# zhaoyuhsin/Edge-Guided-Near-Eye-Image-Analysis-for-Head-Mounted-Displays

Measured on AMD Instinct MI355X. Metric: eye-frames/sec (320x240): inference edge+seg (value), +fit, exact fp32, and train fwd+bwd at 1 MI355X, higher is better.
Workload: dtype f32 tensors; inference products split into f16 hi/lo pairs (3 f16 MFMAs per product, 22-bit significand), f32 accumulate (`exact_fp32`: every product on the f32 MFMA); `train`: bf16 storage, f32 accumulate, f32 master weights (and an f32-storage leg)

## Files before the change

edge-guided-near-eye-image-analysis-for-head-mounted-displays_amd/csrc/common.h:

```cpp
#pragma once
#include <hip/hip_runtime.h>
#include <cstdarg>
#include <cstdio>
#include <mutex>
#include <unordered_map>
#include "../../include/egne_hip.h"

static __device__ __attribute__((aligned(256), used)) float egne_zero_page[64] = {0};

typedef __bf16 egne_bf16;
typedef float egne_f32x4 __attribute__((ext_vector_type(4)));
typedef __bf16 egne_bf16x4 __attribute__((ext_vector_type(4)));
typedef __bf16 egne_bf16x8 __attribute__((ext_vector_type(8)));

__device__ __forceinline__ egne_f32x4 ld4(const float* p) { return *(const egne_f32x4*)p; }
__device__ __forceinline__ egne_f32x4 ld4(const egne_bf16* p) { return __builtin_convertvector(*(const egne_bf16x4*)p, egne_f32x4); }
__device__ __forceinline__ void st4(float* p, egne_f32x4 v) { *(egne_f32x4*)p = v; }
__device__ __forceinline__ void st4(egne_bf16* p, egne_f32x4 v) { *(egne_bf16x4*)p = __builtin_convertvector(v, egne_bf16x4); }
__device__ __forceinline__ float ld1(const float* p) { return *p; }
__device__ __forceinline__ float ld1(const egne_bf16* p) { return (float)*p; }
__device__ __forceinline__ void st1(float* p, float v) { *p = v; }
__device__ __forceinline__ void st1(egne_bf16* p, float v) { *p = (egne_bf16)v; }
template <typename T> struct egne_vt { static constexpr int N = 4; };
template <> struct egne_vt<egne_bf16> { static constexpr int N = 8; };
template <int N> struct egne_fv { float v[N]; };
__device__ __forceinline__ egne_fv<4> ldv(const float* p) {
  const egne_f32x4 t = *(const egne_f32x4*)p;
  return egne_fv<4>{{t[0], t[1], t[2], t[3]}};
}
__device__ __forceinline__ egne_fv<8> ldv(const egne_bf16* p) {
  typedef unsigned u4_ __attribute__((ext_vector_type(4)));
  const u4_ w = *(const u4_*)p;
  egne_fv<8> r;
#pragma unroll
  for (int i = 0; i < 4; ++i) {
    r.v[2 * i] = __builtin_bit_cast(float, w[i] << 16);
    r.v[2 * i + 1] = __builtin_bit_cast(float, w[i] & 0xffff0000u);
  }
  return r;
}
__device__ __forceinline__ void stv(float* p, const egne_fv<4>& a) { *(egne_f32x4*)p = egne_f32x4{a.v[0], a.v[1], a.v[2], a.v[3]}; }
__device__ __forceinline__ void stv(egne_bf16* p, const egne_fv<8>& a) {
  const egne_f32x4 lo = {a.v[0], a.v[1], a.v[2], a.v[3]}, hi = {a.v[4], a.v[5], a.v[6], a.v[7]};
  const egne_bf16x4 l = __builtin_convertvector(lo, egne_bf16x4), h = __builtin_convertvector(hi, egne_bf16x4);
  *(egne_bf16x8*)p = egne_bf16x8{l[0], l[1], l[2], l[3], h[0], h[1], h[2], h[3]};
}
typedef unsigned egne_u32x4 __attribute__((ext_vector_type(4)));
template <typename T> __device__ __forceinline__ egne_u32x4 ldraw(const T* p) { return *(const egne_u32x4*)p; }
__device__ __forceinline__ egne_fv<4> unpackv(const float*, egne_u32x4 w) {
  return egne_fv<4>{{__builtin_bit_cast(float, w[0]), __builtin_bit_cast(float, w[1]), __builtin_bit_cast(float, w[2]), __builtin_bit_cast(float, w[3])}};
}
__device__ __forceinline__ egne_fv<8> unpackv(const egne_bf16*, egne_u32x4 w) {
  egne_fv<8> r;
#pragma unroll
  for (int i = 0; i < 4; ++i) {
    r.v[2 * i] = __builtin_bit_cast(float, w[i] << 16);
    r.v[2 * i + 1] = __builtin_bit_cast(float, w[i] & 0xffff0000u);
  }
  return r;
}
template <int N> __device__ __forceinline__ egne_fv<N> ldf(const float* p) {
  egne_fv<N> r;
#pragma unroll
  for (int i = 0; i < N; i += 4) { const egne_f32x4 t = *(const egne_f32x4*)(p + i); r.v[i] = t[0]; r.v[i + 1] = t[1]; r.v[i + 2] = t[2]; r.v[i + 3] = t[3]; }
  return r;
}
template <int N> __device__ __forceinline__ egne_fv<N> fv_fill(float x) {
  egne_fv<N> r;
#pragma unroll
  for (int i = 0; i < N; ++i) r.v[i] = x;
  return r;
}
template <typename T> __device__ __forceinline__ const T* zero_page() { return (const T*)egne_zero_page; }

#ifdef EGNE_NO_OVF_CHECK
__device__ __forceinline__ bool egne_nonfinite(float) { return false; }
__device__ __forceinline__ bool egne_nonfinite64(double) { return false; }
#else
__device__ __forceinline__ bool egne_nonfinite(float v) { return __builtin_amdgcn_classf(v, 0x207); }
__device__ __forceinline__ bool egne_nonfinite64(double v) { return !__builtin_isfinite(v); }
#endif
__device__ __forceinline__ bool egne_ovf_row(int y, int H) { return y % 3 == 1 || y == H - 1; }
__device__ __forceinline__ void egne_ovf_commit(bool bad, unsigned* flag) {
  if (flag && bad) atomicOr(flag, 1u);
}

namespace egne {

char* err_buf();

inline int fail(int code, const char* fmt, ...) {
  va_list ap;
  va_start(ap, fmt);
  vsnprintf(err_buf(), 512, fmt, ap);
  va_end(ap);
  return code;
}

inline bool fp32_storage(const egne_conv_desc& d) {
  for (int i = 0; i < d.nseg && i < EGNE_MAXSEG; ++i)
    if (d.seg[i].presplit != 0) return false;
  return d.out_split == 0;
}

inline int check_launch(const char* what) {
  hipError_t e = hipGetLastError();
  if (e != hipSuccess) return fail(EGNE_ERR_LAUNCH, "%s: %s", what, hipGetErrorString(e));
  return EGNE_OK;
}

inline bool raise_lds(const void* kern, size_t bytes) {
  static std::mutex mu;
  static std::unordered_map<const void*, size_t> have;
  std::lock_guard<std::mutex> g(mu);
  auto it = have.find(kern);
  if (it != have.end() && it->second >= bytes) return true;
  if (hipFuncSetAttribute(kern, hipFuncAttributeMaxDynamicSharedMemorySize, (int)bytes) != hipSuccess) {
    (void)hipGetLastError();
    return false;
  }
  have[kern] = bytes;
  return true;
}
template <typename... K> inline bool raise_lds_all(size_t bytes, K... kern) { return (raise_lds((const void*)kern, bytes) && ...); }

#define EGNE_REQUIRE(cond, ...) \
  do { if (!(cond)) return ::egne::fail(EGNE_ERR_ARG, __VA_ARGS__); } while (0)

bool halo3_supported(const egne_conv_desc& d);
int halo3_launch(const egne_conv_desc& d, hipStream_t st);

bool wgrad_halo_supported(const egne_conv_desc& d, long long gzs);
int wgrad_halo_splits(const egne_conv_desc& d);
int wgrad_halo_launch(const egne_conv_desc& d, const float* gz, long long gzs, int gzo, float* ws, hipStream_t st);
int wgrad_halo_f16_launch(const egne_conv_desc& d, const float* gz, long long gzs, int gzo, const unsigned* gz_dyn, float* ws, hipStream_t st);

bool wgrad3x3_bf16_supported(const egne_conv_desc& d, long long gzs);
int wgrad3x3_bf16_splits(const egne_conv_desc& d);
int wgrad3x3_bf16_launch(const egne_conv_desc& d, const egne_bf16* gz, long long gzs, int gzo, float* ws, hipStream_t st);
bool wgrad1x1_bf16_supported(const egne_conv_desc& d, long long gzs);
int wgrad1x1_bf16_splits(const egne_conv_desc& d);
int wgrad1x1_bf16_launch(const egne_conv_desc& d, const egne_bf16* gz, long long gzs, int gzo, float* ws, hipStream_t st);

inline int cdiv(long long a, long long b) { return (int)((a + b - 1) / b); }

}
```

edge-guided-near-eye-image-analysis-for-head-mounted-displays_amd/csrc/conv_f16x3_big.hip:

```cpp
#include "common.h"
#include "kernel_util.h"
#include "split_f16.h"
#include <cstdlib>
#include <type_traits>

namespace {

constexpr int BM = 256, ROWB = 128;

template <int NB, bool M16, int NP = 3, int PS = 0>
__global__ __launch_bounds__(512) void conv_f16x3_big_kernel(const egne_conv_desc p, const char* __restrict__ wimg, float a_scale,
                                                             float out_scale) {
  constexpr int BN = 128 * NB;
  constexpr int STAGE = (BM + BN) * ROWB;
  extern __shared__ __attribute__((aligned(1024))) char lds[];
  const int tid = threadIdx.x, lane = tid & 63;
  const int wave = (PS & 2) ? __builtin_amdgcn_readfirstlane(tid >> 6) : tid >> 6;
  const int wm = wave >> 2, wn = wave & 3;
  const long long M = (long long)p.B * p.Ho * p.Wo;
  const long long m0 = (long long)blockIdx.x * BM;
  const int ntile = blockIdx.y;
  const int T = p.kh * p.kw;
  const egne_seg sg = p.seg[0];
  const int hw = p.Ho * p.Wo, frame_px = p.H * p.W;
  const int b0 = (int)(m0 / hw);
  const long long in_left = ((long long)p.B - b0) * frame_px * sg.pix_stride * 4;
  const __amdgpu_buffer_rsrc_t rin = make_rsrc(sg.ptr + (long long)b0 * frame_px * sg.pix_stride,
                                               (unsigned)(in_left < 0x7fffffffll ? in_left : 0x7fffffffll));
  const int nchunk = sg.Cp >> 5;
  const int nsteps = T * nchunk;
  const __amdgpu_buffer_rsrc_t rw = make_rsrc(wimg + (long long)ntile * nsteps * (BN * ROWB), (unsigned)(nsteps * BN * ROWB));

  const int c4 = tid & 7;
  int roff[4];
  unsigned tapmask[4];
  {
    const int dil = p.dil[0];
#pragma unroll
    for (int i = 0; i < 4; ++i) {
      const int row_i = (PS & 2) ? 32 * wave + 8 * i + (lane >> 3) : (tid >> 3) + 64 * i;
      const long long m = m0 + row_i;
      const int b = (int)(m / hw);
      const int r = (int)(m - (long long)b * hw);
      const int oy = r / p.Wo, ox = r - oy * p.Wo;
      const int lc = (lane & 7) ^ (((row_i >> 1) + 6) & 7);
      roff[i] = ((((b - b0) * p.H + oy) * p.W + ox) * (int)sg.pix_stride + sg.ch_off) * 4 + ((PS & 2) ? (lc & 1) * 64 + (lc >> 1) * 16 : c4 * 16);
      unsigned mk = 0;
      for (int ky = 0; ky < p.kh; ++ky)
        for (int kx = 0; kx < p.kw; ++kx) {
          const int iy = oy + (ky - p.pad_h) * dil, ix = ox + (kx - p.pad_w) * dil;
          if (m < M && iy >= 0 && iy < p.H && ix >= 0 && ix < p.W) mk |= 1u << (ky * p.kw + kx);
        }
      tapmask[i] = mk;
    }
  }
  int ldst_hi[4], ldst_lo[4];
#pragma unroll
  for (int i = 0; i < 4; ++i) {
    const int r = (tid >> 3) + 64 * i, g = c4 >> 1, sw = ((r >> 1) + 6) & 7;
    ldst_hi[i] = r * ROWB + (((2 * g) ^ sw) << 4) + (c4 & 1) * 8;
    ldst_lo[i] = r * ROWB + (((2 * g + 1) ^ sw) << 4) + (c4 & 1) * 8;
  }
  const int wvoff = lane * 16;

  u32x4 ra[4];
  int ky_n = 0, kx_n = 0, c0_n = 0;
  auto load_a = [&](int tap, int stage) {
    const int dil = p.dil[0];
    const int tapoff = (((ky_n - p.pad_h) * p.W + (kx_n - p.pad_w)) * dil * (int)sg.pix_stride + c0_n) * 4;
#pragma unroll
    for (int i = 0; i < 4; ++i) {
      const bool ok = (tapmask[i] >> tap) & 1u;
      if constexpr ((PS & 2))
        __builtin_amdgcn_raw_ptr_buffer_load_lds(rin, (lds_ptr)(lds + stage * STAGE + wave * 4096 + i * 1024), 16, ok ? roff[i] + tapoff : (int)OOB, 0, 0, 0);
      else
        ra[i] = __builtin_amdgcn_raw_buffer_load_b128(rin, ok ? roff[i] + tapoff : (int)OOB, 0, 0);
    }
  };
  auto dma_b = [&](int stage, int step) {
    char* base = lds + stage * STAGE + BM * ROWB;
#pragma unroll
    for (int j = 0; j < 2 * NB; ++j) {
      const int blk = wave * 2 * NB + j;
      __builtin_amdgcn_raw_ptr_buffer_load_lds(rw, (lds_ptr)(base + blk * 1024), 16, wvoff, step * (BN * ROWB) + blk * 1024, 0, 0);
    }
  };
  auto store_a = [&](int stage) {
    char* base = lds + stage * STAGE;
#pragma unroll
    for (int i = 0; i < ((PS & 2) ? 0 : 4); ++i) {
      const f32x4 v = __builtin_bit_cast(f32x4, ra[i]);
      if constexpr (NP == 1) {
        const f32x2 t0 = {v[0] * a_scale, v[1] * a_scale}, t1 = {v[2] * a_scale, v[3] * a_scale};
        const h2 h0 = __builtin_convertvector(t0, h2), h1 = __builtin_convertvector(t1, h2);
        const h4 hi = {h0[0], h0[1], h1[0], h1[1]};
        *(h4*)(base + ldst_hi[i]) = hi;
        continue;
      }
      h2 h0, h1, l0, l1;
      egne::split2(v[0], v[1], a_scale, h0, l0);
      egne::split2(v[2], v[3], a_scale, h1, l1);
      const h4 hi = {h0[0], h0[1], h1[0], h1[1]}, lo = {l0[0], l0[1], l1[0], l1[1]};
      *(h4*)(base + ldst_hi[i]) = hi;
      *(h4*)(base + ldst_lo[i]) = lo;
    }
  };
  auto advance = [&]() {
    if (++kx_n == p.kw) { kx_n = 0; ++ky_n; }
    if (ky_n == p.kh) { ky_n = 0; c0_n += 32; }
  };

  constexpr int MB = M16 ? 16 : 32, NTM = 128 / MB, NTN = 32 * NB / MB;
  using acc_t = std::conditional_t<M16, f32x4, f32x16>;
  acc_t acc[NTM][NTN];
#pragma unroll
  for (int a = 0; a < NTM; ++a)
#pragma unroll
    for (int b = 0; b < NTN; ++b) acc[a][b] = (acc_t)(0.f);

  const int lr = lane & (MB - 1), kg = lane / MB;
  int aoffs[NTM], boffs[NTN];
#pragma unroll
  for (int t = 0; t < NTM; ++t) aoffs[t] = (wm * 128 + t * MB + lr) * ROWB;
#pragma unroll
  for (int t = 0; t < NTN; ++t) boffs[t] = BM * ROWB + (wn * 32 * NB + t * MB + lr) * ROWB;
  const int sw = ((lr >> 1) + 6) & 7;

  load_a(0, 0);
  dma_b(0, 0);
  store_a(0);
  advance();
  asm volatile("s_waitcnt vmcnt(0) lgkmcnt(0)" ::: "memory");
  __builtin_amdgcn_s_barrier();

  int tap_n = 1 % T;
  for (int step = 0; step < nsteps; ++step) {
    const int st = step & 1;
    const bool more = step + 1 < nsteps;
    if (more) {
      load_a(tap_n, st ^ 1);
      dma_b(st ^ 1, step + 1);
    }
    const char* base = lds + st * STAGE;
    if constexpr (M16) {
      const int ch = ((2 * kg) ^ sw) << 4, cl = ((2 * kg + 1) ^ sw) << 4;
      h8 bh[NTN], bl[NTN];
#pragma unroll
      for (int t = 0; t < NTN; ++t) {
        bh[t] = *(const h8*)(base + boffs[t] + ch);
        if constexpr (NP == 3) bl[t] = *(const h8*)(base + boffs[t] + cl);
      }
#pragma unroll
      for (int half = 0; half < 2; ++half) {
        h8 ah[4], al[4];
#pragma unroll
        for (int t = 0; t < 4; ++t) {
          ah[t] = *(const h8*)(base + aoffs[half * 4 + t] + ch);
          if constexpr (NP == 3) al[t] = *(const h8*)(base + aoffs[half * 4 + t] + cl);
        }
#pragma unroll
        for (int t = 0; t < 4; ++t)
#pragma unroll
          for (int tn = 0; tn < NTN; ++tn) {
            acc_t& c = acc[half * 4 + t][tn];
            if constexpr (NP == 3) {
              c = __builtin_amdgcn_mfma_f32_16x16x32_f16(bh[tn], al[t], c, 0, 0, 0);
              c = __builtin_amdgcn_mfma_f32_16x16x32_f16(bl[tn], ah[t], c, 0, 0, 0);
            }
            c = __builtin_amdgcn_mfma_f32_16x16x32_f16(bh[tn], ah[t], c, 0, 0, 0);
          }
      }
    } else {
#pragma unroll
    for (int ks = 0; ks < 2; ++ks) {
      const int ch = ((2 * (2 * ks + kg)) ^ sw) << 4, cl = ((2 * (2 * ks + kg) + 1) ^ sw) << 4;
      h8 ah[4], al[4], bh[NB], bl[NB];
#pragma unroll
      for (int t = 0; t < 4; ++t) {
        ah[t] = *(const h8*)(base + aoffs[t] + ch);
        al[t] = *(const h8*)(base + aoffs[t] + cl);
      }
#pragma unroll
      for (int t = 0; t < NB; ++t) {
        bh[t] = *(const h8*)(base + boffs[t] + ch);
        bl[t] = *(const h8*)(base + boffs[t] + cl);
      }
#pragma unroll
      for (int tm = 0; tm < 4; ++tm)
#pragma unroll
        for (int tn = 0; tn < NB; ++tn) {
          if constexpr (!M16) {
            acc[tm][tn] = __builtin_amdgcn_mfma_f32_32x32x16_f16(bh[tn], al[tm], acc[tm][tn], 0, 0, 0);
            acc[tm][tn] = __builtin_amdgcn_mfma_f32_32x32x16_f16(bl[tn], ah[tm], acc[tm][tn], 0, 0, 0);
            acc[tm][tn] = __builtin_amdgcn_mfma_f32_32x32x16_f16(bh[tn], ah[tm], acc[tm][tn], 0, 0, 0);
          }
        }
    }
    }
    if (more) {
      store_a(st ^ 1);
      advance();
      tap_n = tap_n + 1 == T ? 0 : tap_n + 1;
    }
    asm volatile("s_waitcnt vmcnt(0) lgkmcnt(0)" ::: "memory");
    __builtin_amdgcn_s_barrier();
  }

  const float slope = p.act == EGNE_ACT_RELU ? 0.f : (p.act == EGNE_ACT_LEAKY ? 0.01f : 1.f);
  const long long left = M - m0;
  const __amdgpu_buffer_rsrc_t rout = make_rsrc(p.out + m0 * p.out_pix_stride, (unsigned)((left < BM ? left : BM) * p.out_pix_stride * 4));
  constexpr int NJ = M16 ? 1 : 4;
  bool bad = false;
  if constexpr (PS & 1) {
    static_assert(M16 && NP == 3, "split-pair output: 16 x 16 x 32 shape, three products");
    const float oss = p.out_split_scale;
    const bool odd = kg & 1;
    const int pb = (odd ? 32 : 0) + 16 * (kg >> 1);
#pragma unroll
    for (int bp = 0; bp < NTN / 2; ++bp) {
      const int nb = ntile * BN + wn * 32 * NB + bp * 32;
      const bool nok = nb < p.Cout_store;
      const f32x4 bv0 = (p.bias && nok) ? *(const f32x4*)(p.bias + nb + 4 * kg) : (f32x4)(0.f);
      const f32x4 bv1 = (p.bias && nok) ? *(const f32x4*)(p.bias + nb + 16 + 4 * kg) : (f32x4)(0.f);
#pragma unroll
      for (int tm = 0; tm < NTM; ++tm) {
        u32x2 hi[2], lo[2];
#pragma unroll
        for (int q = 0; q < 2; ++q) {
          f32x4 v;
#pragma unroll
          for (int e = 0; e < 4; ++e) {
            const float t = acc[tm][2 * bp + q][e] * out_scale + (q ? bv1[e] : bv0[e]);
            v[e] = fmaxf(t, t * slope);
          }
          h2 h0, h1, l0, l1;
          egne::split2(v[0], v[1], oss, h0, l0);
          egne::split2(v[2], v[3], oss, h1, l1);
          if (bp == 0 && q == 0) bad |= egne_nonfinite(v[0]) || egne_nonfinite((float)h0[0]);
          hi[q] = u32x2{__builtin_bit_cast(unsigned, h0), __builtin_bit_cast(unsigned, h1)};
          lo[q] = u32x2{__builtin_bit_cast(unsigned, l0), __builtin_bit_cast(unsigned, l1)};
        }
        const u32x2 sh = odd ? hi[0] : hi[1], sl = odd ? lo[0] : lo[1];
        u32x2 rh, rl;
#pragma unroll
        for (int e = 0; e < 2; ++e) {
          rh[e] = (unsigned)__builtin_amdgcn_ds_swizzle((int)sh[e], 0x401f);
          rl[e] = (unsigned)__builtin_amdgcn_ds_swizzle((int)sl[e], 0x401f);
        }
        const u32x4 oh = odd ? u32x4{rh[0], rh[1], hi[1][0], hi[1][1]} : u32x4{hi[0][0], hi[0][1], rh[0], rh[1]};
        const u32x4 ol = odd ? u32x4{rl[0], rl[1], lo[1][0], lo[1][1]} : u32x4{lo[0][0], lo[0][1], rl[0], rl[1]};
        const int row = wm * 128 + tm * MB + lr;
        const int o = nok ? (row * (int)p.out_pix_stride + p.out_ch_off + nb) * 4 + pb : (int)OOB;
        __builtin_amdgcn_raw_buffer_store_b128(oh, rout, o, 0, 0);
        __builtin_amdgcn_raw_buffer_store_b128(ol, rout, o + 64, 0, 0);
      }
    }
    egne_ovf_commit(bad, p.ovf_flag);
    return;
  }
#pragma unroll
  for (int tn = 0; tn < NTN; ++tn)
#pragma unroll
    for (int j = 0; j < NJ; ++j) {
      const int n = ntile * BN + wn * 32 * NB + tn * MB + (M16 ? 4 * kg : 8 * j + 4 * kg);
      const bool nok = n < p.Cout_store;
      const f32x4 bv = (p.bias && nok) ? *(const f32x4*)(p.bias + n) : (f32x4)(0.f);
#pragma unroll
      for (int tm = 0; tm < NTM; ++tm) {
        f32x4 v;
#pragma unroll
        for (int e = 0; e < 4; ++e) {
          const float t = acc[tm][tn][4 * j + e] * out_scale + bv[e];
          v[e] = fmaxf(t, t * slope);
        }
        if (tn == 0 && j == 0) bad |= egne_nonfinite(v[0]);
        const int row = wm * 128 + tm * MB + lr;
        __builtin_amdgcn_raw_buffer_store_b128(__builtin_bit_cast(u32x4, v), rout,
                                               nok ? (row * (int)p.out_pix_stride + p.out_ch_off + n) * 4 : (int)OOB, 0, 0);
      }
    }
  egne_ovf_commit(bad, p.ovf_flag);
}

__global__ void pack_weight_f16img_k(const float* __restrict__ w, int Cout, int Cin, int T, int BN, int ntiles, int nchunk,
                                     float wscale, _Float16* __restrict__ out) {
  const long long total = (long long)ntiles * nchunk * T * BN * 64;
  for (long long i = (long long)blockIdx.x * blockDim.x + threadIdx.x; i < total; i += (long long)gridDim.x * blockDim.x) {
    const int e = (int)(i & 7), pc = (int)((i >> 3) & 7);
    long long q = i >> 6;
    const int j = (int)(q % BN); q /= BN;
    const int step = (int)(q % (nchunk * T));
    const int nt = (int)(q / (nchunk * T));
    const int chunk = step / T, tap = step - chunk * T;
    const int lc = pc ^ (((j >> 1) + 6) & 7), g = lc >> 1, hl = lc & 1;
    const int n = nt * BN + j, ci = chunk * 32 + 8 * g + e;
    const float v = (n < Cout && ci < Cin) ? w[((long long)n * Cin + ci) * T + tap] * wscale : 0.f;
    const _Float16 h = (_Float16)v;
    out[i] = hl ? (_Float16)(v - (float)h) : h;
  }
}

}

extern "C" int egne_pack_conv_weight_f16img(const float* w_oihw, int Cout, int Cin, int kh, int kw, int BN, int Ktot, float wscale,
                                            void* wimg, void* stream) {
  EGNE_REQUIRE(w_oihw && wimg && Cout > 0 && Cin > 0 && (BN == 128 || BN == 256) && Ktot >= Cin && Ktot % 32 == 0 && wscale > 0.f,
               "pack_f16img: bad sizes Cout %d Cin %d BN %d Ktot %d", Cout, Cin, BN, Ktot);
  const int ntiles = (Cout + BN - 1) / BN, nchunk = Ktot / 32;
  long long total = (long long)ntiles * nchunk * kh * kw * BN * 64, g = (total + 255) / 256;
  if (g > 8192) g = 8192;
  hipLaunchKernelGGL(pack_weight_f16img_k, dim3((unsigned)g), dim3(256), 0, (hipStream_t)stream, w_oihw, Cout, Cin, kh * kw, BN, ntiles,
                     nchunk, wscale, (_Float16*)wimg);
  return egne::check_launch("egne_pack_conv_weight_f16img");
}

extern "C" int egne_conv2d_f16x3_big_fwd(const egne_conv_desc* dp, const void* wimg, float a_scale, float w_scale, void* stream) {
  EGNE_REQUIRE(dp && wimg, "conv_f16x3_big: null pointer");
  const egne_conv_desc& d = *dp;
  EGNE_REQUIRE(d.nseg == 1 && d.ngroups == 1 && d.stride == 1 && d.pad_mode == 0 && !d.seg[0].scale && !d.seg[0].shift && !d.residual &&
               !d.post_scale, "conv_f16x3_big: unsupported descriptor");
  EGNE_REQUIRE(d.kh >= 1 && d.kw >= 1 && d.kh * d.kw <= 32, "conv_f16x3_big: %d taps (%dx%d): the per-row tap mask holds 32", d.kh * d.kw, d.kh, d.kw);
  const egne_seg& g = d.seg[0];
  EGNE_REQUIRE(g.ptr && g.Cp % 32 == 0 && g.Cp == d.Ktot && ((uintptr_t)g.ptr & 15) == 0 && g.ch_off % 4 == 0 && g.pix_stride % 4 == 0,
               "conv_f16x3_big: input slice (Cp %d Ktot %d)", g.Cp, d.Ktot);
  EGNE_REQUIRE(d.CoutP % 128 == 0 && d.Cout_store <= d.CoutP && d.Cout_store % 4 == 0 && d.out && ((uintptr_t)d.out & 15) == 0 &&
               d.out_ch_off % 4 == 0 && d.out_pix_stride % 4 == 0 && d.out_ch_off + d.Cout_store <= d.out_pix_stride &&
               d.out_pix_stride * 1024 < (1ll << 31) && (!d.bias || ((uintptr_t)d.bias & 15) == 0), "conv_f16x3_big: output");
  const int dd = d.dil[0];
  EGNE_REQUIRE(dd >= 1 && d.H + 2 * d.pad_h * dd - dd * (d.kh - 1) == d.Ho && d.W + 2 * d.pad_w * dd - dd * (d.kw - 1) == d.Wo,
               "conv_f16x3_big: output %dx%d inconsistent with geometry", d.Ho, d.Wo);
  EGNE_REQUIRE(((uintptr_t)wimg & 15) == 0 && a_scale > 0.f && w_scale > 0.f, "conv_f16x3_big: weights / scales");
  EGNE_REQUIRE((g.presplit == 0 || g.presplit == 3) && (d.out_split == 0 || d.out_split == 3),
               "conv_f16x3_big: storage (presplit %d, out_split %d): 0 or 3 (channel-order split pairs)", g.presplit, d.out_split);
  const long long M = (long long)d.B * d.Ho * d.Wo;
  const float os = 1.0f / (a_scale * w_scale);
  hipStream_t st = (hipStream_t)stream;
  if (d.out_split == 3 || g.presplit == 3) {
    EGNE_REQUIRE(d.f16_products != 1 && (d.out_split == 0 || (d.out_split_scale > 0.f && d.Cout_store % 32 == 0 && d.out_ch_off % 32 == 0)) &&
                 (g.presplit == 0 || g.ch_off % 32 == 0), "conv_f16x3_big: split-pair slices are whole 32-channel blocks, three products");
    const bool in3 = g.presplit == 3, out3 = d.out_split == 3;
#define EGNE_BIGP_GO(NBV, PSV)                                                                                                               \
  do {                                                                                                                                      \
    if (!egne::raise_lds((const void*)conv_f16x3_big_kernel<NBV, true, 3, PSV>, 2 * (BM + 128 * NBV) * ROWB))                               \
      return egne::fail(EGNE_ERR_LAUNCH, "conv_f16x3_big: cannot raise the dynamic LDS limit");                                             \
    hipLaunchKernelGGL((conv_f16x3_big_kernel<NBV, true, 3, PSV>), dim3((unsigned)((M + BM - 1) / BM), (unsigned)(d.CoutP / (128 * NBV))),  \
                       dim3(512), 2 * (BM + 128 * NBV) * ROWB, st, d, (const char*)wimg, a_scale, os);                                      \
  } while (0)
    if (d.CoutP % 256 == 0) { if (in3 && out3) EGNE_BIGP_GO(2, 3); else if (in3) EGNE_BIGP_GO(2, 2); else EGNE_BIGP_GO(2, 1); }
    else { if (in3 && out3) EGNE_BIGP_GO(1, 3); else if (in3) EGNE_BIGP_GO(1, 2); else EGNE_BIGP_GO(1, 1); }
#undef EGNE_BIGP_GO
    return egne::check_launch("egne_conv2d_f16x3_big_fwd");
  }
  static const bool m16 = !(getenv("EGNE_BIG_M16") && atoi(getenv("EGNE_BIG_M16")) == 0);
  if (!egne::raise_lds((const void*)conv_f16x3_big_kernel<2, false>, 128 * 1024) || !egne::raise_lds((const void*)conv_f16x3_big_kernel<1, false>, 96 * 1024) ||
      !egne::raise_lds((const void*)conv_f16x3_big_kernel<2, true>, 128 * 1024) || !egne::raise_lds((const void*)conv_f16x3_big_kernel<1, true>, 96 * 1024))
    return egne::fail(EGNE_ERR_LAUNCH, "conv_f16x3_big: cannot raise the dynamic LDS limit");
  if (d.f16_products == 1) {
    if (!egne::raise_lds((const void*)conv_f16x3_big_kernel<2, true, 1>, 128 * 1024) || !egne::raise_lds((const void*)conv_f16x3_big_kernel<1, true, 1>, 96 * 1024))
      return egne::fail(EGNE_ERR_LAUNCH, "conv_f16x3_big: cannot raise the dynamic LDS limit");
    if (d.CoutP % 256 == 0)
      hipLaunchKernelGGL((conv_f16x3_big_kernel<2, true, 1>), dim3((unsigned)((M + BM - 1) / BM), (unsigned)(d.CoutP / 256)), dim3(512), 2 * (BM + 256) * ROWB, st, d, (const char*)wimg, a_scale, os);
    else
      hipLaunchKernelGGL((conv_f16x3_big_kernel<1, true, 1>), dim3((unsigned)((M + BM - 1) / BM), (unsigned)(d.CoutP / 128)), dim3(512), 2 * (BM + 128) * ROWB, st, d, (const char*)wimg, a_scale, os);
    return egne::check_launch("egne_conv2d_f16x3_big_fwd");
  }
  if (d.CoutP % 256 == 0) {
    dim3 grid((unsigned)((M + BM - 1) / BM), (unsigned)(d.CoutP / 256));
    if (m16) hipLaunchKernelGGL((conv_f16x3_big_kernel<2, true>), grid, dim3(512), 2 * (BM + 256) * ROWB, st, d, (const char*)wimg, a_scale, os);
    else hipLaunchKernelGGL((conv_f16x3_big_kernel<2, false>), grid, dim3(512), 2 * (BM + 256) * ROWB, st, d, (const char*)wimg, a_scale, os);
  } else {
    dim3 grid((unsigned)((M + BM - 1) / BM), (unsigned)(d.CoutP / 128));
    if (m16) hipLaunchKernelGGL((conv_f16x3_big_kernel<1, true>), grid, dim3(512), 2 * (BM + 128) * ROWB, st, d, (const char*)wimg, a_scale, os);
    else hipLaunchKernelGGL((conv_f16x3_big_kernel<1, false>), grid, dim3(512), 2 * (BM + 128) * ROWB, st, d, (const char*)wimg, a_scale, os);
  }
  return egne::check_launch("egne_conv2d_f16x3_big_fwd");
}
```

Measured before the change: 2206.

## Add ring-buffered LDS pipeline for presplit-input big f16x3 conv kernel

For presplit input (PS&2), the big f16x3 conv kernel now uses a new main loop. A tiles are double-buffered through direct buffer-to-LDS loads, B (weight) tiles go through a three-slot ring, and B fragments for the next step are read from LDS while the current step's MFMAs run. The aim is to hide global-to-LDS latency and cut register staging. The cost is more LDS per block, which may lower occupancy. raise_lds now also keys its cache per device, which is a correctness fix for multi-GPU use.

```diff
diff --git a/edge-guided-near-eye-image-analysis-for-head-mounted-displays_amd/csrc/common.h b/edge-guided-near-eye-image-analysis-for-head-mounted-displays_amd/csrc/common.h
--- a/edge-guided-near-eye-image-analysis-for-head-mounted-displays_amd/csrc/common.h
+++ b/edge-guided-near-eye-image-analysis-for-head-mounted-displays_amd/csrc/common.h
@@ -2,8 +2,10 @@
 #include <hip/hip_runtime.h>
 #include <cstdarg>
 #include <cstdio>
+#include <map>
 #include <mutex>
 #include <unordered_map>
+#include <utility>
 #include "../../include/egne_hip.h"
 
 static __device__ __attribute__((aligned(256), used)) float egne_zero_page[64] = {0};
@@ -111,15 +113,21 @@
 
 inline bool raise_lds(const void* kern, size_t bytes) {
   static std::mutex mu;
-  static std::unordered_map<const void*, size_t> have;
+  static std::map<std::pair<int, const void*>, size_t> have;
+  int dev = 0;
+  if (hipGetDevice(&dev) != hipSuccess) {
+    (void)hipGetLastError();
+    return false;
+  }
   std::lock_guard<std::mutex> g(mu);
-  auto it = have.find(kern);
+  const auto key = std::make_pair(dev, kern);
+  auto it = have.find(key);
   if (it != have.end() && it->second >= bytes) return true;
   if (hipFuncSetAttribute(kern, hipFuncAttributeMaxDynamicSharedMemorySize, (int)bytes) != hipSuccess) {
     (void)hipGetLastError();
     return false;
   }
-  have[kern] = bytes;
+  have[key] = bytes;
   return true;
 }
 template <typename... K> inline bool raise_lds_all(size_t bytes, K... kern) { return (raise_lds((const void*)kern, bytes) && ...); }
diff --git a/edge-guided-near-eye-image-analysis-for-head-mounted-displays_amd/csrc/conv_f16x3_big.hip b/edge-guided-near-eye-image-analysis-for-head-mounted-displays_amd/csrc/conv_f16x3_big.hip
--- a/edge-guided-near-eye-image-analysis-for-head-mounted-displays_amd/csrc/conv_f16x3_big.hip
+++ b/edge-guided-near-eye-image-analysis-for-head-mounted-displays_amd/csrc/conv_f16x3_big.hip
@@ -126,6 +126,95 @@
   for (int t = 0; t < NTN; ++t) boffs[t] = BM * ROWB + (wn * 32 * NB + t * MB + lr) * ROWB;
   const int sw = ((lr >> 1) + 6) & 7;
 
+  if constexpr ((PS & 2) != 0) {
+    static_assert(M16 && NP == 3, "ring form: 16 x 16 x 32 shape, three products");
+    constexpr int ASLOT = BM * ROWB, BSLOT = BN * ROWB, BBASE = 2 * ASLOT, NVB = 2 * NB;
+    static_assert(BBASE + 3 * BSLOT <= 163840, "LDS budget");
+    int tap_r = 0;
+    auto ring_a = [&](int slot, bool on) {
+      const int dil = p.dil[0];
+      const int tapoff = (((ky_n - p.pad_h) * p.W + (kx_n - p.pad_w)) * dil * (int)sg.pix_stride + c0_n) * 4;
+      char* base = lds + slot * ASLOT + wave * 4096;
+#pragma unroll
+      for (int i = 0; i < 4; ++i) {
+        const bool ok = on && ((tapmask[i] >> tap_r) & 1u);
+        __builtin_amdgcn_raw_ptr_buffer_load_lds(rin, (lds_ptr)(base + i * 1024), 16, ok ? roff[i] + tapoff : (int)OOB, 0, 0, 0);
+      }
+      advance();
+      tap_r = tap_r + 1 == T ? 0 : tap_r + 1;
+    };
+    auto ring_b = [&](int slot, int step) {
+      const int s = step < nsteps ? step : nsteps - 1;
+      char* base = lds + BBASE + slot * BSLOT;
+#pragma unroll
+      for (int j = 0; j < NVB; ++j) {
+        const int blk = wave * NVB + j;
+        __builtin_amdgcn_raw_ptr_buffer_load_lds(rw, (lds_ptr)(base + blk * 1024), 16, wvoff, s * BSLOT + blk * 1024, 0, 0);
+      }
+    };
+    const int ch = ((2 * kg) ^ sw) << 4, cl = ((2 * kg + 1) ^ sw) << 4;
+    const int a_lane = (wm * 128 + lr) * ROWB, b_lane = BBASE + (wn * 32 * NB + lr) * ROWB;
+    auto read_a = [&](h8* h, h8* l, int slot, int half) {
+      const char* base = lds + slot * ASLOT + a_lane + half * 64 * ROWB;
+#pragma unroll
+      for (int t = 0; t < 4; ++t) {
+        l[t] = *(const h8*)(base + t * 16 * ROWB + cl);
+        h[t] = *(const h8*)(base + t * 16 * ROWB + ch);
+      }
+    };
+    auto read_b1 = [&](h8* h, h8* l, int slot, int t) {
+      const char* base = lds + slot * BSLOT + b_lane + t * 16 * ROWB;
+      h[t] = *(const h8*)(base + ch);
+      l[t] = *(const h8*)(base + cl);
+    };
+    auto mfma_block = [&](const h8* ah, const h8* al, const h8* bh, const h8* bl, int half, int t) {
+#pragma unroll
+      for (int tn = 0; tn < NTN; ++tn) {
+        acc_t& c = acc[half * 4 + t][tn];
+        c = __builtin_amdgcn_mfma_f32_16x16x32_f16(bh[tn], al[t], c, 0, 0, 0);
+        c = __builtin_amdgcn_mfma_f32_16x16x32_f16(bl[tn], ah[t], c, 0, 0, 0);
+        c = __builtin_amdgcn_mfma_f32_16x16x32_f16(bh[tn], ah[t], c, 0, 0, 0);
+      }
+    };
+
+    h8 ah[2][4], al[2][4], bh[2][NTN], bl[2][NTN];
+    ring_a(0, true);
+    ring_b(0, 0);
+    ring_b(1, 1);
+    ring_b(2, 2);
+    asm volatile("s_waitcnt vmcnt(%0)" ::"n"(NVB) : "memory");
+    __builtin_amdgcn_s_barrier();
+#pragma unroll
+    for (int t = 0; t < NTN; ++t) read_b1(bh[0], bl[0], 0, t);
+    asm volatile("s_waitcnt lgkmcnt(0)" ::: "memory");
+    __builtin_amdgcn_s_barrier();
+    int s3 = 0;
+    auto step_body = [&](int step, auto pc) {
+      constexpr int P = decltype(pc)::value;
+      const int s3n = s3 == 2 ? 0 : s3 + 1;
+      ring_a(P ^ 1, step + 1 < nsteps);
+      ring_b(s3, step + 3);
+      read_a(ah[0], al[0], P, 0);
+      read_a(ah[1], al[1], P, 1);
+#pragma unroll
+      for (int t = 0; t < 4; ++t) mfma_block(ah[0], al[0], bh[P], bl[P], 0, t);
+#pragma unroll
+      for (int t = 0; t < 4; ++t) {
+        __builtin_amdgcn_sched_barrier(0);
+        if (2 * t < NTN) read_b1(bh[P ^ 1], bl[P ^ 1], s3n, 2 * t);
+        if (2 * t + 1 < NTN) read_b1(bh[P ^ 1], bl[P ^ 1], s3n, 2 * t + 1);
+        mfma_block(ah[1], al[1], bh[P], bl[P], 1, t);
+      }
+      s3 = s3n;
+      asm volatile("s_waitcnt vmcnt(%0) lgkmcnt(0)" ::"n"(NVB) : "memory");
+      __builtin_amdgcn_s_barrier();
+    };
+    for (int step = 0; step < nsteps; step += 2) {
+      step_body(step, std::integral_constant<int, 0>{});
+      if (step + 1 < nsteps) step_body(step + 1, std::integral_constant<int, 1>{});
+    }
+    asm volatile("s_waitcnt vmcnt(0)" ::: "memory");
+  } else {
   load_a(0, 0);
   dma_b(0, 0);
   store_a(0);
@@ -204,6 +293,7 @@
     }
     asm volatile("s_waitcnt vmcnt(0) lgkmcnt(0)" ::: "memory");
     __builtin_amdgcn_s_barrier();
+  }
   }
 
   const float slope = p.act == EGNE_ACT_RELU ? 0.f : (p.act == EGNE_ACT_LEAKY ? 0.01f : 1.f);
@@ -341,10 +431,11 @@
     const bool in3 = g.presplit == 3, out3 = d.out_split == 3;
 #define EGNE_BIGP_GO(NBV, PSV)                                                                                                               \
   do {                                                                                                                                      \
-    if (!egne::raise_lds((const void*)conv_f16x3_big_kernel<NBV, true, 3, PSV>, 2 * (BM + 128 * NBV) * ROWB))                               \
+    constexpr int lds_bytes = ((PSV) & 2) ? (2 * BM + 3 * 128 * NBV) * ROWB : 2 * (BM + 128 * NBV) * ROWB;                                  \
+    if (!egne::raise_lds((const void*)conv_f16x3_big_kernel<NBV, true, 3, PSV>, lds_bytes))                                                 \
       return egne::fail(EGNE_ERR_LAUNCH, "conv_f16x3_big: cannot raise the dynamic LDS limit");                                             \
     hipLaunchKernelGGL((conv_f16x3_big_kernel<NBV, true, 3, PSV>), dim3((unsigned)((M + BM - 1) / BM), (unsigned)(d.CoutP / (128 * NBV))),  \
-                       dim3(512), 2 * (BM + 128 * NBV) * ROWB, st, d, (const char*)wimg, a_scale, os);                                      \
+                       dim3(512), lds_bytes, st, d, (const char*)wimg, a_scale, os);                                                        \
   } while (0)
     if (d.CoutP % 256 == 0) { if (in3 && out3) EGNE_BIGP_GO(2, 3); else if (in3) EGNE_BIGP_GO(2, 2); else EGNE_BIGP_GO(2, 1); }
     else { if (in3 && out3) EGNE_BIGP_GO(1, 3); else if (in3) EGNE_BIGP_GO(1, 2); else EGNE_BIGP_GO(1, 1); }
```

New measurement: 2218 (median of 6 runs). Within noise of the previous version (+0.5%).
